# nordmtr/quantpy

Hardware: AMD Instinct MI355X
Metric: state reconstructions/sec (3-qubit MLE) (higher is better)
Workload: dtype f64

## Files before the change

quantpy_amd/csrc/qt_linesearch.h:

```cpp
#pragma once
#include <math.h>

#if defined(__HIPCC__)
#include <hip/hip_runtime.h>
#define QT_HD __host__ __device__ __forceinline__
#else
#define QT_HD inline
#endif

namespace qt {

enum LsResult : int { LS_EVAL = 0, LS_ACCEPT = 1, LS_FAIL = 2 };

struct LineSearch {
  double phi0, old_phi0, derphi0;
  int mode;
  int brackt, stage, evals;
  double gtest, width, width1, stx, fx, gx, sty, fy, gy, stmin, stmax;
  double alpha0, alpha1, phi_a0, phi_a1, derphi_a0;
  int it;
  double a_lo, a_hi, phi_lo, phi_hi, derphi_lo, phi_rec, a_rec;
  int zi;

  static constexpr double C1 = 1e-4, C2 = 0.9, AMAX = 1e100, AMIN = 1e-100, XTOL = 1e-14;
// ... 183 lines not shown
    }
    if (brackt) {
      if (fabs(sty - stx) >= 0.66 * width1) stp = stx + 0.5 * (sty - stx);
      width1 = width;
      width = fabs(sty - stx);
      stmin = dmin(stx, sty);
      stmax = dmax(stx, sty);
    } else {
      stmin = stp + 1.1 * (stp - stx);
      stmax = stp + 4.0 * (stp - stx);
    }
    stp = dmin(dmax(stp, AMIN), AMAX);
    if ((brackt && (stp <= stmin || stp >= stmax)) || (brackt && stmax - stmin <= XTOL * stmax)) stp = stx;
    if (!isfinite(stp)) return LS_FAIL;
    if (evals >= 99) return LS_FAIL;
    *next = stp;
    return LS_EVAL;
  }

  QT_HD static double cubicmin(double a, double fa, double fpa, double b, double fb, double c, double fc) {
    const double C = fpa, db = b - a, dc = c - a;
    const double denom = (db * dc) * (db * dc) * (db - dc);
    if (denom == 0.0) return NAN;
    const double t0 = fb - fa - C * db, t1 = fc - fa - C * dc;
    double A = dc * dc * t0 - db * db * t1;
    double B = -(dc * dc * dc) * t0 + db * db * db * t1;
    A /= denom;
    B /= denom;
    const double radical = B * B - 3.0 * A * C;
    if (!(radical >= 0.0) || A == 0.0) return NAN;
    const double x = a + (-B + sqrt(radical)) / (3.0 * A);
    return isfinite(x) ? x : NAN;
  }

  QT_HD static double quadmin(double a, double fa, double fpa, double b, double fb) {
    const double db = b - a;
    if (db == 0.0) return NAN;
    const double B = (fb - fa - fpa * db) / (db * db);
    if (B == 0.0) return NAN;
    const double x = a - fpa / (2.0 * B);
    return isfinite(x) ? x : NAN;
  }

  QT_HD int zoom_begin(double alo, double ahi, double plo, double phi_h, double dlo, double* next) {
    mode = 2;
    a_lo = alo; a_hi = ahi; phi_lo = plo; phi_hi = phi_h; derphi_lo = dlo;
    phi_rec = phi0;
    a_rec = 0.0;
    zi = 0;
    return zoom_propose(next);
  }

  QT_HD int zoom_propose(double* next) {
    const double dalpha = a_hi - a_lo;
    double a = a_lo, b = a_hi;
    if (dalpha < 0.0) { a = a_hi; b = a_lo; }
    double aj = NAN;
    bool need_quad = true;
    if (zi > 0) {
      const double cchk = 0.2 * dalpha;
      aj = cubicmin(a_lo, phi_lo, derphi_lo, a_hi, phi_hi, a_rec, phi_rec);
      need_quad = isnan(aj) || aj > b - cchk || aj < a + cchk;
    }
    if (need_quad) {
      const double qchk = 0.1 * dalpha;
      aj = quadmin(a_lo, phi_lo, derphi_lo, a_hi, phi_hi);
      if (isnan(aj) || aj > b - qchk || aj < a + qchk) aj = a_lo + 0.5 * dalpha;
    }
    *next = aj;
    return LS_EVAL;
  }

  QT_HD int advance_fallback(double stp, double f, double g, double* next) {
    if (mode == 1) {
      phi_a1 = f;
      const double derphi_a1 = g;
      if (alpha1 == 0.0 || alpha0 > AMAX) return LS_FAIL;
      if (phi_a1 > phi0 + C1 * alpha1 * derphi0 || (phi_a1 >= phi_a0 && it > 0))
        return zoom_begin(alpha0, alpha1, phi_a0, phi_a1, derphi_a0, next);
      if (fabs(derphi_a1) <= -C2 * derphi0) return LS_ACCEPT;
      if (derphi_a1 >= 0.0) return zoom_begin(alpha1, alpha0, phi_a1, phi_a0, derphi_a1, next);
      const double alpha2 = dmin(2.0 * alpha1, AMAX);
      alpha0 = alpha1;
      alpha1 = alpha2;
      phi_a0 = phi_a1;
      derphi_a0 = derphi_a1;
      ++it;
      if (it >= 10) mode = 3;
      *next = alpha1;
      return LS_EVAL;
    }
    if (mode == 3) return LS_ACCEPT;
    const double a_j = stp, phi_aj = f, derphi_aj = g;
    if (phi_aj > phi0 + C1 * a_j * derphi0 || phi_aj >= phi_lo) {
      phi_rec = phi_hi; a_rec = a_hi;
      a_hi = a_j; phi_hi = phi_aj;
    } else {
      if (fabs(derphi_aj) <= -C2 * derphi0) return LS_ACCEPT;
      if (derphi_aj * (a_hi - a_lo) >= 0.0) {
        phi_rec = phi_hi; a_rec = a_hi;
        a_hi = a_lo; phi_hi = phi_lo;
      } else {
        phi_rec = phi_lo; a_rec = a_lo;
      }
      a_lo = a_j; phi_lo = phi_aj; derphi_lo = derphi_aj;
    }
    ++zi;
    if (zi > 10) return LS_FAIL;
    return zoom_propose(next);
  }
};


enum TrialStatus : int {
  TRIAL_OK = 0,
  TRIAL_NOT_PD = 1,
  TRIAL_LINESEARCH = 2,
  TRIAL_MAXITER = 3,
  TRIAL_NAN = 4,
  TRIAL_SHOTS = 5
};

QT_HD int bfgs_eval_cap(int max_iter) { return (max_iter + 2) * 130; }

QT_HD double bfgs_rho(double ys) { return ys == 0.0 ? 1000.0 : 1.0 / ys; }

QT_HD bool bfgs_step_exit(double gnorm, double gtol, double stp, double pnorm2, double fk, int kiter, int max_iter,
                          int* status) {
  if (gnorm <= gtol) return true;
  if (stp * sqrt(pnorm2) <= 0.0) return true;
  if (!isfinite(fk)) {
    *status = TRIAL_LINESEARCH;
    return true;
  }
  return !(gnorm > gtol && kiter < max_iter);
}

QT_HD int bfgs_final_status(int status, int kiter, int max_iter, double gn, double fk, double xn) {
  if (status != TRIAL_OK) return status;
  if (kiter >= max_iter) return TRIAL_MAXITER;
  if (gn != gn || fk != fk || xn != xn) return TRIAL_NAN;
  return TRIAL_OK;
}

QT_HD int mle_start_status(bool shots_ok, bool ok, bool iterate, int max_iter, double gnorm, double fk, bool xnan) {
  if (!shots_ok) return TRIAL_SHOTS;
  if (!ok) return TRIAL_NOT_PD;
  if (iterate) return TRIAL_OK;
  if (0 >= max_iter) return TRIAL_MAXITER;
  if (gnorm != gnorm || fk != fk || xnan) return TRIAL_NAN;
  return TRIAL_OK;
}

}
```

quantpy_amd/csrc/qt_mle_small.h:

```cpp
#pragma once
#include <hip/hip_runtime.h>
#include <stdint.h>

#include <type_traits>

#include "qt_linesearch.h"
#include "qt_small.h"

namespace qt {

template <int NQ, bool GENERIC>
constexpr bool kStartBallots = NQ == 3 && !GENERIC && kLaneLeftovers;
template <int G>
__device__ __forceinline__ double start_norm_ballots(double gk, double gtol, bool& above) {
  const bool nan = group_any<G>(gk != gk);
  above = !nan && group_any<G>(fabs(gk) > gtol);
  return nan ? __builtin_nan("") : 0.0;
}

template <int NQ, bool GENERIC>
__global__ void __launch_bounds__(256) __attribute__((amdgpu_waves_per_eu(4))) k_mle_start(const int64_t* __restrict__ counts, const void* image, const double* Ns, int B, int M, int extra,
                                                   int max_iter, double gtol, typename MleArgs<GENERIC>::type pv0, int init, EstOut rho,
                                                   int32_t* __restrict__ nit_out, int32_t* __restrict__ nfev_out,
                                                   double* __restrict__ fun_out, int32_t* __restrict__ status_out,
// ... 235 lines not shown
    return -q;
  }
};

template <int NQ, class C>
__device__ __forceinline__ void bfgs_iterate(const C& c, bool mine, double xk, double gk,
                                             double fk, int b, int max_iter, double gtol, EstOut rho,
                                             int32_t* __restrict__ nit_out, int32_t* __restrict__ nfev_out,
                                             double* __restrict__ fun_out, int32_t* __restrict__ status_out) {
  DenseH<NQ> dir(c);
  LineSearch ls;
  bfgs_loop<NQ>(c, dir, ls, mine, xk, gk, fk, b, max_iter, gtol, rho, nit_out, nfev_out, fun_out, status_out);
}

template <int NQ, int LP = 0, class C>
__device__ __forceinline__ void bfgs_iterate_2l(const C& c, bool mine, double xk, double gk,
                                                double fk, int b, int max_iter, double gtol, EstOut rho,
                                                int32_t* __restrict__ nit_out, int32_t* __restrict__ nfev_out,
                                                double* __restrict__ fun_out, int32_t* __restrict__ status_out,
                                                double* __restrict__ pairs) {
  TwoLoop<NQ, LP> dir(c, pairs, b, max_iter);
  static_assert(sizeof(LineSearch) <= LineSearch::SLOTS * sizeof(double), "LDS slot of the line-search state");
  LineSearch& ls = *reinterpret_cast<LineSearch*>(c.extra());
  bfgs_loop<NQ>(c, dir, ls, mine, xk, gk, fk, b, max_iter, gtol, rho, nit_out, nfev_out, fun_out, status_out);
}

#ifndef QT_BFGS_WAVES
#define QT_BFGS_WAVES 2
#endif
template <int NQ, bool GENERIC>
__global__ void __launch_bounds__(256) __attribute__((amdgpu_waves_per_eu(QT_BFGS_WAVES))) k_mle_bfgs(const int64_t* __restrict__ counts, const void* image, const double* Ns, int B, int M, int extra, int max_iter,
                                                  double gtol, typename MleArgs<GENERIC>::type pv0, EstOut rho, int32_t* __restrict__ nit_out,
                                                  int32_t* __restrict__ nfev_out, double* __restrict__ fun_out,
                                                  int32_t* __restrict__ status_out, const double* __restrict__ ws_x,
                                                  const double* __restrict__ ws_g, const double* __restrict__ ws_f,
                                                  const int32_t* __restrict__ ws_active, double* __restrict__ pairs) {
  using S = Small<NQ>;
  constexpr int D = S::D;
  bool live;
  const int b = S::trial_index(B, &live);
  const bool mine = live && ws_active[b] != 0;
  if (!__syncthreads_or(mine)) return;
  extern __shared__ __attribute__((aligned(16))) double smem[];
  std::conditional_t<GENERIC, typename S::Ctx, typename S::template CtxSV<0>> c;
  const int bb = live ? b : B - 1;
  const auto pv = mle_front(pv0, image, Ns, M, extra);
  if constexpr (GENERIC) {
    S::make_ctx(c, smem, pv);
    S::load_freq(c, counts + (size_t)bb * pv.M);
  } else {
    typename S::Prefetch pf;
    S::prefetch_counts(pf, counts + (size_t)bb * pv.M, pv);
    S::take_coefs(c, pv);
    S::make_ctx(c, smem, pv, pf);
    S::load_freq(c, pf);
  }
  const double xk = mine ? ws_x[(size_t)b * D + c.l] : (c.l < S::d ? 1.0 : 0.0);
  const double gk = mine ? ws_g[(size_t)b * D + c.l] : 0.0;
  const double fk = mine ? ws_f[b] : 0.0;
  if constexpr (NQ == 3)
    bfgs_iterate_2l<NQ>(c, mine, xk, gk, fk, b, max_iter, gtol, rho, nit_out, nfev_out, fun_out, status_out, pairs);
  else
    bfgs_iterate<NQ>(c, mine, xk, gk, fk, b, max_iter, gtol, rho, nit_out, nfev_out, fun_out, status_out);
}

constexpr int kFusedLdsPairs = 24;
constexpr int kFusedHwLdsPairs = 16;

template <int NQ, bool GENERIC, bool HW = false>
__device__ __forceinline__ void mle_fused_body(const typename MleArgs<GENERIC>::type& pv, const int64_t* __restrict__ counts, int B, int init,
                                               int max_iter, double gtol, EstOut rho,
                                               int32_t* __restrict__ nit_out, int32_t* __restrict__ nfev_out,
                                               double* __restrict__ fun_out, int32_t* __restrict__ status_out,
                                               double* __restrict__ pairs) {
  using S = Small<NQ>;
  constexpr int D = S::D, G = S::G, d = S::d;
  extern __shared__ __attribute__((aligned(16))) double smem[];
  using Ctx = std::conditional_t<GENERIC, typename S::Ctx, typename S::template CtxSV<2>>;
  std::conditional_t<HW, typename S::template WithHelper<Ctx>, Ctx> c;
  [[maybe_unused]] typename S::HelperLink link;
  [[maybe_unused]] typename S::LateX late{false, 0.0, 0};
  [[maybe_unused]] int twin = 0;
  [[maybe_unused]] double* trial_sm = nullptr;
  bool live;
  const int b = S::trial_index(B, &live);
  const int bb = live ? b : B - 1;
  typename S::Prefetch pf;
  S::prefetch_counts(pf, counts + (size_t)bb * pv.M, pv);
  if constexpr (!GENERIC) S::take_coefs(c, pv);
  if constexpr (HW) {
    static_assert(NQ == 3, "one trial per wavefront");
    static_assert(S::HelperLink::doubles() <= kFusedHwLdsPairs * 2 * D, "the hand-off lives in the LDS pair store");
    int r1 = 6;
    if constexpr (GENERIC) r1 = pv.pr.R1;
    const int per_trial = S::trial_doubles(pv.M, r1);
    trial_sm = smem + S::table_doubles(pv.M, r1) + (threadIdx.x >> 6) * (per_trial + pv.extra);
    link.base = trial_sm + per_trial + LineSearch::SLOTS + 2 * max_iter;
    twin = __builtin_amdgcn_readfirstlane((int)threadIdx.y);
    link.pending = 0;
    if (!twin) link.reset();
    if (twin) __builtin_amdgcn_s_setprio(1);
    c.link = &link;
    c.xtra = trial_sm + per_trial;
    c.late = &late;
  }
  bool shots_ok;
  if constexpr (GENERIC) {
    S::template make_ctx<HW>(c, smem, pv, twin);
    QT_STAMP(0);
    shots_ok = S::load_freq(c, counts + (size_t)bb * pv.M, &pf);
  } else {
    S::template make_ctx<true, HW>(c, smem, pv, pf, twin);
    QT_STAMP(0);
    shots_ok = S::load_freq(c, pf);
  }
  QT_STAMP(1);
  int ok;
  double xk;
  typename S::StartPoint sp;
  [[maybe_unused]] cd lin;
  if (init == 0) {
    double bl;
    lin = S::lin_invert(c, bl);
    QT_STAMP(2);
    bool feasible = false;
    if constexpr (HW) {
      if (twin) {
        if (!S::twin_lift(c, link, lin, sp.rho)) {
          S::HelperLink::publish(link.gone(), 1);
          return;
        }
        sp.lscale = 1.0;
        link.pending = 1;
        feasible = true;
      }
    }
    if (!feasible) sp.rho = S::template make_feasible<!HW>(c, lin, &xk, &ok, &sp.lscale);
    if constexpr (HW) {
      if (!twin && __builtin_amdgcn_readfirstlane(link.pending)) {
        int r1 = 6;
        if constexpr (GENERIC) r1 = pv.pr.R1;
        double* twin_sm = smem + S::twin_offset(pv.M, r1, pv.extra) + (threadIdx.x >> 6) * S::trial_doubles(pv.M, r1);
        S::sweep_for(c, link, sp.rho, reinterpret_cast<cd*>(twin_sm + S::oB));
        S::HelperLink::publish(link.gone(), 1);
        return;
      }
    }
  } else {
    sp.rho = cd{c.i == c.j ? 1.0 / d : 0.0, 0.0};
    sp.lscale = 1.0;
    xk = S::cholesky_param(c, sp.rho, ok);
  }
  QT_STAMP(8);
  double fk, gk;
  cd rho_l;
  [[maybe_unused]] typename S::DeferredValue dv;
  bool evaluate = true;
  if constexpr (HW) {
    if (__builtin_amdgcn_readfirstlane(link.pending)) {
      if constexpr (GENERIC) S::template nll_grad<false, decltype(c), true>(c, 0.0, fk, gk, &rho_l, true, &sp);
      else S::template nll_grad<true, decltype(c), true>(c, 0.0, fk, gk, &rho_l, true, &sp, &dv);
      xk = late.x;
      ok = late.ok;
      const bool got = __builtin_amdgcn_readfirstlane((int)late.got) != 0;
      if (!got) xk = S::cholesky_param(c, sp.rho, ok);
      ok = __builtin_amdgcn_readfirstlane(ok);
      evaluate = !got || !ok;
      if (!ok) {
        sp.rho = S::psd_project(c, lin, 1e-15);
        xk = S::cholesky_param(c, sp.rho, ok);
      }
    }
  }
  if (evaluate) {
    if constexpr (GENERIC) S::nll_grad(c, xk, fk, gk, &rho_l, true, &sp);
    else S::template nll_grad<true>(c, xk, fk, gk, &rho_l, true, &sp, &dv);
  }
  double gnorm;
  bool iterate;
  if constexpr (kStartBallots<NQ, GENERIC>) {
    bool above;
    gnorm = start_norm_ballots<G>(gk, gtol, above);
    QT_STAMP(9);
    iterate = live && shots_ok && ok && above && (0 < max_iter);
  } else {
    gnorm = gmax<G>(fabs(gk));
    QT_STAMP(9);
    iterate = live && shots_ok && ok && (gnorm > gtol) && (0 < max_iter);
  }
  if constexpr (!GENERIC) fk = S::value_if_needed(c, dv, iterate || fun_out != nullptr);
  S::emit(c, rho, b, live && !iterate, rho_l);
  const int status = mle_start_status(shots_ok, ok, iterate, max_iter, gnorm, fk, group_any<G>(xk != xk));
  if (live && !iterate && c.l == 0) store_trial(b, 0, ok ? 1 : 0, fk, status, nit_out, nfev_out, fun_out, status_out);
  QT_STAMP(10);
  if (!__any(iterate)) return;
  if (!iterate) {
    xk = (c.l < d) ? 1.0 : 0.0;
    gk = 0.0;
    fk = 0.0;
  }
  if constexpr (HW) link.await_gone();
  if constexpr (NQ == 3)
    bfgs_iterate_2l<NQ, HW ? kFusedHwLdsPairs : kFusedLdsPairs>(c, iterate, xk, gk, fk, b, max_iter, gtol, rho, nit_out, nfev_out, fun_out,
                                              status_out, pairs);
  else
    bfgs_iterate<NQ>(c, iterate, xk, gk, fk, b, max_iter, gtol, rho, nit_out, nfev_out, fun_out, status_out);
}

template <int NQ, bool GENERIC>
__global__ void __launch_bounds__(256) k_mle_fused(const int64_t* __restrict__ counts, const void* image, const double* Ns, int B, int M, int extra, int max_iter,
                                                   double gtol, typename MleArgs<GENERIC>::type pv, EstOut rho, int32_t* __restrict__ nit_out,
                                                   int32_t* __restrict__ nfev_out, double* __restrict__ fun_out,
                                                   int32_t* __restrict__ status_out, double* __restrict__ pairs) {
  mle_fused_body<NQ, GENERIC>(mle_front(pv, image, Ns, M, extra), counts, B, 0, max_iter, gtol, rho, nit_out, nfev_out, fun_out, status_out, pairs);
}
template <int NQ, bool GENERIC>
__global__ void __launch_bounds__(256) k_mle_fused_mixed(const int64_t* __restrict__ counts, const void* image, const double* Ns, int B, int M, int extra,
                                                         int max_iter, double gtol, typename MleArgs<GENERIC>::type pv, EstOut rho,
                                                         int32_t* __restrict__ nit_out, int32_t* __restrict__ nfev_out,
                                                         double* __restrict__ fun_out, int32_t* __restrict__ status_out,
                                                         double* __restrict__ pairs) {
  mle_fused_body<NQ, GENERIC>(mle_front(pv, image, Ns, M, extra), counts, B, 1, max_iter, gtol, rho, nit_out, nfev_out, fun_out, status_out, pairs);
}

template <int NQ, bool GENERIC>
__global__ void __launch_bounds__(512) k_mle_fused_hw(const int64_t* __restrict__ counts, const void* image, const double* Ns, int B, int M, int extra, int max_iter,
                                                      double gtol, typename MleArgs<GENERIC>::type pv, EstOut rho, int32_t* __restrict__ nit_out,
                                                      int32_t* __restrict__ nfev_out, double* __restrict__ fun_out,
                                                      int32_t* __restrict__ status_out, double* __restrict__ pairs) {
  mle_fused_body<NQ, GENERIC, true>(mle_front(pv, image, Ns, M, extra), counts, B, 0, max_iter, gtol, rho, nit_out, nfev_out, fun_out, status_out, pairs);
}

}
```

quantpy_amd/csrc/qt_small.h:

```cpp
#pragma once
#include <hip/hip_runtime.h>
#include <stdint.h>

#include "qt_args.h"
#include "qt_wave.h"

namespace qt {

constexpr bool kLiftSingleNegative = true;

#ifndef QT_LANE_INT_FRONT
#define QT_LANE_INT_FRONT 1
#endif
#ifndef QT_LANE_LEFTOVERS
#define QT_LANE_LEFTOVERS 1
#endif
constexpr bool kLaneLeftovers = QT_LANE_LEFTOVERS != 0;

template <int NQ>
struct Small {
  static constexpr int d = 1 << NQ;
  static constexpr int D = d * d;
  static constexpr int G = D;
  static constexpr int TPW = 64 / G;
  static constexpr int WPB = 4;
  static constexpr int NT = 64 * WPB;
  static constexpr int TPB = TPW * WPB;
  static constexpr int T = d * (d - 1) / 2;
  static constexpr int LD = d == 8 ? 9 : d;
  static constexpr int MAT = 2 * LD * d;
  static constexpr int oA = 0;
  static constexpr int oB = oA + MAT;
  static constexpr int oVec = oB + MAT;
  static constexpr int oLam = oVec + D + 2;
  static constexpr int oM = oLam + 2 * ((d + 1) / 2);
  __host__ __device__ static bool v_on_rbuf(int M) { return ((M + 1) & ~1) >= MAT; }
  __host__ __device__ static int v_offset(int M, int R1) {
    const int Mp = (M + 1) & ~1;
    return v_on_rbuf(M) ? oM : oM + (R1 > 0 ? 3 : 2) * Mp;
  }
  __host__ __device__ static int trial_doubles(int M, int R1 = 0) {
    const int Mp = (M + 1) & ~1;
    return oM + (R1 > 0 ? 3 : 2) * Mp + (v_on_rbuf(M) ? 0 : MAT);
  }
  __host__ __device__ static int ipow_h(int b, int e) {
    int r = 1;
    for (int t = 0; t < e; ++t) r *= b;
    return r;
  }
  __host__ __device__ static int fwd_ints(int R1) {
    int t = 0;
    for (int q = 1; q <= NQ; ++q) t += ipow_h(R1, q) << (2 * (NQ - q));
    return t;
  }
  __host__ __device__ static int bwd_ints(int R1) {
    int t = 0;
    for (int q = 1; q <= NQ; ++q) t += ipow_h(R1, q - 1) << (2 * (NQ - q + 1));
    return t;
  }
  __host__ __device__ static int table_ints(int M, int R1) { return (fwd_ints(R1) + bwd_ints(R1) + M + 1) & ~1; }
  __host__ __device__ static int table_doubles(int M, int R1) {
    return R1 > 0 ? (table_ints(M, R1) / 2 + ((M + 1) & ~1) + 8 * R1) : 0;
  }
  __host__ __device__ static size_t lds_bytes(int M, int R1 = 0, int extra = 0) {
    return ((size_t)table_doubles(M, R1) + (size_t)TPB * (trial_doubles(M, R1) + extra)) * sizeof(double);
  }
  __host__ __device__ static int twin_offset(int M, int R1, int extra) {
    return table_doubles(M, R1) + TPB * (trial_doubles(M, R1) + extra);
  }
  __host__ __device__ static size_t lds_bytes_twin(int M, int R1, int extra) {
    return lds_bytes(M, R1, extra) + (size_t)TPB * trial_doubles(M, R1) * sizeof(double);
  }

  struct Ctx {
    int l, i, j, e;
    double* sm;
    const int *tfwd, *tbwd, *trmap;
    const double* twrow;
    const double *ttab, *ptab;
    int M, Mp;
    PovmView pv;
    int xm, zm, ny;
    int pi, pj, pkind;
    int src_re, src_im;
    __device__ __forceinline__ cd* A() const { return reinterpret_cast<cd*>(sm + oA); }
    __device__ __forceinline__ cd* Bm() const { return reinterpret_cast<cd*>(sm + oB); }
    __device__ __forceinline__ cd* V() const { return reinterpret_cast<cd*>(sm + v_offset(M, pv.pr.enabled ? pv.pr.R1 : 0)); }
    __device__ __forceinline__ double* vec() const { return sm + oVec; }
    __device__ __forceinline__ double* lam() const { return sm + oLam; }
    __device__ __forceinline__ double* rbuf() const { return sm + oM; }
    __device__ __forceinline__ double* freq() const { return sm + oM + Mp; }
    __device__ __forceinline__ double* bufB() const { return sm + oM + 2 * Mp; }
    __device__ __forceinline__ const double* tabT() const { return ttab; }
    __device__ __forceinline__ const double* tabP() const { return ptab; }
    __device__ __forceinline__ bool prod() const { return pv.pr.enabled != 0; }
    __device__ __forceinline__ double* extra() const { return sm + trial_doubles(M, pv.pr.enabled ? pv.pr.R1 : 0); }
    static constexpr bool kGeneric = true;
    static constexpr int kLaneTables = 0;
    static constexpr bool kHelper = false;
    __device__ __forceinline__ static constexpr int verdict_load() { return 0; }
    __device__ __forceinline__ static constexpr bool abandoned(int) { return false; }
    __device__ __forceinline__ int R1() const { return pv.pr.R1; }
    __device__ __forceinline__ bool uniform() const { return pv.pr.uniform != 0; }
    __device__ __forceinline__ bool pairedT() const { return pv.pr.pairedT != 0; }
    __device__ __forceinline__ bool pairedP() const { return pv.pr.pairedP != 0; }
    __device__ __forceinline__ double wuni() const { return pv.pr.wuni; }
    __device__ __forceinline__ double jtol2() const { return pv.jtol2; }
    __device__ __forceinline__ double cT(int k) const { return pv.pr.cT[k]; }
    __device__ __forceinline__ double cP(int k) const { return pv.pr.cP[k]; }
  };
  template <int LT>
  struct CtxSV {
    static constexpr bool VC = LT == 2;
    int l, i, j, e;
    double* sm;
    const int* tfwd;
    const double *ttab, *ptab;
    int M, Mp;
    SpecArgs a;
    int xm, zm, ny;
    int pi, pj, pkind;
    int src_re, src_im;
    int bslot;
    double kT[12], kP[12];
    uint32_t mpack[2];
    const double* mterm[VC ? d : 1];
    uint32_t msign[VC ? d : 1];
    uint32_t bflip[VC ? 4 : 1];
    static constexpr int kLaneTables = LT;
    __device__ __forceinline__ cd* A() const { return reinterpret_cast<cd*>(sm + oA); }
    __device__ __forceinline__ cd* Bm() const { return reinterpret_cast<cd*>(sm + oB); }
    __device__ __forceinline__ cd* V() const { return reinterpret_cast<cd*>(sm + v_offset(M, 6)); }
    __device__ __forceinline__ double* vec() const { return sm + oVec; }
    __device__ __forceinline__ double* lam() const { return sm + oLam; }
    __device__ __forceinline__ double* rbuf() const { return sm + oM; }
    __device__ __forceinline__ double* freq() const { return sm + oM + Mp; }
    __device__ __forceinline__ double* bufB() const { return sm + oM + 2 * Mp; }
    __device__ __forceinline__ const double* tabT() const { return ttab; }
    __device__ __forceinline__ const double* tabP() const { return ptab; }
    __device__ __forceinline__ double* extra() const { return sm + trial_doubles(M, 6); }
    static constexpr bool kGeneric = false;
    static constexpr bool kHelper = false;
    __device__ __forceinline__ static constexpr int verdict_load() { return 0; }
    __device__ __forceinline__ static constexpr bool abandoned(int) { return false; }
    __device__ __forceinline__ static constexpr bool prod() { return true; }
    __device__ __forceinline__ static constexpr int R1() { return 6; }
    __device__ __forceinline__ static constexpr bool uniform() { return true; }
    __device__ __forceinline__ static constexpr bool pairedT() { return true; }
    __device__ __forceinline__ static constexpr bool pairedP() { return true; }
    __device__ __forceinline__ double wuni() const { return a.wuni; }
    __device__ __forceinline__ double jtol2() const { return a.jtol2; }
    __device__ __forceinline__ double cT(int k) const { return kT[k]; }
    __device__ __forceinline__ double cP(int k) const { return kP[k]; }
  };
  using CtxS = CtxSV<1>;
  __device__ __forceinline__ static double pin_vgpr(double x) {
    asm volatile("" : "+v"(x));
    return x;
  }
  template <bool GENERIC, class = void>
  struct CtxOf {
    using type = Ctx;
  };
  template <class X>
  struct CtxOf<false, X> {
    using type = CtxSV<1>;
  };
  __host__ __device__ static int image_last_ints(int M) { return (M + 3) & ~3; }
  __host__ __device__ static int image_chunks(int M) { return image_last_ints(M) / 4 + 2 * 24 / 2; }

// ... 1077 lines not shown
    const int* verdict;
    __device__ __forceinline__ cd* A() const { return image; }
    __device__ __forceinline__ cd* Bm() const { return factor; }
    __device__ __forceinline__ cd* V() const { return second; }
    __device__ __forceinline__ int verdict_load() const {
      return __hip_atomic_load(verdict, __ATOMIC_RELAXED, __HIP_MEMORY_SCOPE_WORKGROUP);
    }
    __device__ __forceinline__ static bool abandoned(int v) {
      v = __builtin_amdgcn_readfirstlane(v);
      return v != HelperLink::kPending && v != HelperLink::kGo;
    }
  };
  struct LateX {
    bool got;
    double x;
    int ok;
  };
  template <class Base>
  struct WithHelper : Base {
    HelperLink* link;
    LateX* late;
    double* xtra;
    __device__ __forceinline__ double* extra() const { return xtra; }
    static constexpr bool kHelper = true;
  };
  __device__ __forceinline__ static void param_owner(int l, int& pi, int& pj, int& pkind) {
    const bool diag = l < d, imag = l >= d + T;
    const int t = l - d - (imag ? T : 0);
    int ii = 1;
#pragma unroll
    for (int k = 2; k < d; ++k) ii += t >= (k * (k - 1)) / 2;
    pkind = diag ? 0 : imag ? 2 : 1;
    pi = diag ? l : ii;
    pj = diag ? l : t - (ii * (ii - 1)) / 2;
  }
  template <class C>
  __device__ static bool twin_lift(const C& t, const HelperLink& k, cd lin, cd& proj) {
    static_assert(G == 64, "one trial per wavefront");
    CtxH c = side_ctx(t, k, t.Bm());
    proj = cd{0.0, 0.0};
    const bool lifted = __builtin_amdgcn_readfirstlane((int)lift_single_negative<true>(c, lin, d - 1, 1e-15, proj, nullptr)) != 0;
    QT_STAMP(6);
    if (HelperLink::template poll<1>(k.verdict(), HelperLink::kPending, HelperLink::kHelperPolls) != HelperLink::kGo) return false;
    QT_STAMP(7);
    if (!HelperLink::claim(k.verdict(), HelperLink::kGo, HelperLink::kClaimed)) return false;
    if (!lifted) {
      HelperLink::publish(k.lifted(), HelperLink::kRefused);
      return false;
    }
    k.result()[c.e] = proj;
    HelperLink::publish(k.lifted(), HelperLink::kLifted);
    return true;
  }
  template <class C>
  __device__ static void sweep_for(const C& t, const HelperLink& k, cd proj, cd* L) {
    CtxH c = side_ctx(t, k, L);
    int ok2;
    const double x2 = cholesky_param(c, proj, ok2);
    k.x()[c.l] = x2;
    if (c.l == 0) *k.ok() = ok2;
    HelperLink::publish(k.done(), 1);
    QT_STAMP(7);
  }
  template <class C>
  __device__ __forceinline__ static CtxH side_ctx(const C& t, const HelperLink& k, cd* L) {
    CtxH c;
    c.l = t.l;
    c.i = t.i;
    c.j = t.j;
    c.e = t.e;
    c.pi = t.pi;
    c.pj = t.pj;
    c.pkind = t.pkind;
    c.image = t.A();
    c.second = t.V();
    c.factor = L;
    c.verdict = k.verdict();
    return c;
  }

  template <bool NATURAL = false, class C>
  __device__ static bool lift_single_negative(const C& c, cd r, int kneg, double eps, cd& out,
                                              const cd* inverse = nullptr) {
    static_assert(G == 64, "one trial per wavefront: the flags below are wave-uniform");
    cd* Ai = c.A();
    cd* Vi = c.V();
    const int i = c.i, j = c.j;
    if (i == j) r.im = 0.0;
    cd b = r;
    if (inverse) b = *inverse;
    auto eliminate = [&](int p) {
      Ai[c.e] = b;
      const double piv = readlane_f64(b.re, p * d + p);
      wave_sync();
      const cd bip = Ai[i * LD + p], bpj = Ai[p * LD + j];
      wave_sync();
      double inv = __builtin_amdgcn_rcp(piv);
      inv = fma(inv, fma(-piv, inv, 1.0), inv);
      inv = fma(inv, fma(-piv, inv, 1.0), inv);
      const cd t{bpj.re * inv, bpj.im * inv};
      const cd e = cmul(bip, t);
      cd nb{b.re - e.re, b.im - e.im};
      if (j == p) nb = cd{-bip.re * inv, -bip.im * inv};
      if (i == p) nb = (j == p) ? cd{inv, 0.0} : t;
      b = nb;
    };
    if constexpr (NATURAL) {
      if (!inverse) {
#pragma unroll
        for (int p = 0; p < d; ++p) eliminate(p);
      }
    } else {
#pragma unroll 1
      for (int s = inverse ? d : 0; s < d; ++s) eliminate(s < kneg ? s : (s < d - 1 ? s + 1 : kneg));
    }
    QT_STAMP(4);
    b = cscale(b, fast_rsqrt(gsum<G>(b.re * b.re + b.im * b.im)));
    bool certified = false, called_off = false;
#pragma unroll 1
    for (int k = 1;; ++k) {
      Ai[c.e] = b;
      wave_sync();
      [[maybe_unused]] const int verdict = c.verdict_load();
      cd n{0.0, 0.0}, n2{0.0, 0.0};
#pragma unroll
      for (int q = 0; q < d; q += 2) {
        const cd u = Ai[i * LD + q], v = Ai[j * LD + q];
        n.re = fma(u.re, v.re, fma(u.im, v.im, n.re));
        n.im = fma(u.im, v.re, fma(-u.re, v.im, n.im));
        if (q + 1 < d) {
          const cd u2 = Ai[i * LD + q + 1], v2 = Ai[j * LD + q + 1];
          n2.re = fma(u2.re, v2.re, fma(u2.im, v2.im, n2.re));
          n2.im = fma(u2.im, v2.re, fma(-u2.re, v2.im, n2.im));
        }
      }
      n = cadd(n, n2);
      wave_sync();
      called_off = c.abandoned(verdict);
      const double pur = gsum<G>(n.re * n.re + n.im * n.im);
      b = cscale(n, fast_rsqrt(pur));
      const double defect = 1.0 - pur;
      QT_STAMP_VAL(20, k);
#ifdef QT_PHASE_TIMING
      if (k <= 5) QT_STAMP(25 + k);
#endif
      if (called_off | certified | (k == 7) | ((k == 3) & !(defect < 0.05))) break;
      certified = defect < 1e-7;
    }
    QT_STAMP(5);
    if (called_off || !certified) return false;
    if (i == j) b.im = 0.0;
    b = cscale(b, 1.0 / gtrace<G>(i == j, b.re));
    const double lam = gsum<G>(r.re * b.re + r.im * b.im);
    if (!(lam < eps)) return false;
    Ai[c.e] = r;
    Vi[c.e] = b;
    wave_sync();
    cd q{-lam * b.re, -lam * b.im};
#pragma unroll
    for (int k = 0; k < d; ++k) {
      const cd u = Ai[i * LD + k], v = Vi[j * LD + k];
      q.re = fma(u.re, v.re, fma(u.im, v.im, q.re));
      q.im = fma(u.im, v.re, fma(-u.re, v.im, q.im));
    }
    wave_sync();
    const double res2 = gsum<G>(q.re * q.re + q.im * q.im);
    const double nrm2 = gsum<G>(r.re * r.re + r.im * r.im);
    if (!(res2 <= 1e-26 * nrm2)) return false;
    const double w = eps - lam;
    cd o{fma(w, b.re, r.re), fma(w, b.im, r.im)};
    const double tr = gtrace<G>(i == j, o.re);
    out = cd{o.re / tr, o.im / tr};
    return true;
  }

  template <bool SPEC = false, class C>
  __device__ static cd make_feasible(const C& c, cd r, double* xl, int* ok_out, double* lscale_out = nullptr) {
    int ok, neg, kneg;
    cd spec_inv{0.0, 0.0};
    double x = cholesky_param<SPEC && G == 64>(c, r, ok, &neg, &kneg, &spec_inv);
    QT_STAMP(3);
    cd out{0.0, 0.0};
    double lscale = 1.0;
    auto pd_epilogue = [&]() {
      const double tr = gtrace<G>(c.i == c.j, r.re);
      out = cd{r.re / tr, r.im / tr};
      const double rst = tr > 0.0 ? fast_rsqrt(tr) : 1.0 / sqrt(tr);
      x = x * rst;
      lscale = rst;
    };
    const bool all_pd = __all(ok);
    [[maybe_unused]] bool go = false;
    if constexpr (C::kHelper) {
      go = kLiftSingleNegative && !all_pd && __builtin_amdgcn_readfirstlane(neg) == 1 &&
           __builtin_amdgcn_readfirstlane(kneg) == d - 1;
      c.link->decide(go);
    }
    if (G < 64 || all_pd || (!xl && lscale_out)) pd_epilogue();
    if (!all_pd) {
      cd proj;
      bool lifted = false;
      [[maybe_unused]] bool refused = false;
      if constexpr (C::kHelper) {
        if (go) {
          const int came = c.link->await_lift(c.e, proj);
          QT_STAMP(31);
          if (came == HelperLink::kLifted) {
            QT_STAMP(6);
            if (lscale_out) *lscale_out = 1.0;
            return proj;
          }
          refused = came == HelperLink::kRefused;
        }
      }
      if constexpr (G == 64) {
        if (kLiftSingleNegative && !refused && __builtin_amdgcn_readfirstlane(neg) == 1) {
          const int kn = __builtin_amdgcn_readfirstlane(kneg);
          lifted = __builtin_amdgcn_readfirstlane(
                       (int)lift_single_negative(c, r, kn, 1e-15, proj, SPEC && kn == d - 1 ? &spec_inv : nullptr)) != 0;
        }
      }
      if (!lifted) proj = psd_project(c, r, 1e-15);
      QT_STAMP(6);
      int ok2 = 1;
      double x2 = xl ? cholesky_param(c, proj, ok2) : 0.0;
      if (lifted && xl && !__all(ok2 || ok)) {
        proj = psd_project(c, r, 1e-15);
        x2 = cholesky_param(c, proj, ok2);
      }
      QT_STAMP(7);
      if (xl) lscale = 1.0;
      if (!ok) {
        out = proj;
        x = x2;
        ok = ok2;
      }
    }
    if (xl) *xl = x;
    if (ok_out) *ok_out = ok;
    if (lscale_out) *lscale_out = lscale;
    return out;
  }

  template <class C>
  __device__ static cd build_llh(const C& c, double xl, double& tr) {
    double* vx = c.vec();
    cd* L = c.Bm();
    vx[c.l] = xl;
    tr = gsum<G>(xl * xl);
    wave_sync();
    const int i = c.i, j = c.j;
    L[c.e] = cd{vx[c.src_re], vx[c.src_im]};
    wave_sync();
    cd m{0.0, 0.0};
#pragma unroll
    for (int k = 0; k < d; ++k) {
      const cd u = L[i * LD + k], v = L[j * LD + k];
      m.re = fma(u.re, v.re, fma(u.im, v.im, m.re));
      m.im = fma(u.im, v.re, fma(-u.re, v.im, m.im));
    }
    return m;
  }

  struct StartPoint {
    cd rho;
    double lscale;
  };
  template <bool DEFER = false, class C, bool LATE = false>
  __device__ static void nll_grad(const C& c, double xl, double& f, double& gl, cd* rho_l = nullptr,
                                  bool want_grad = true, const StartPoint* start = nullptr, DeferredValue* dv = nullptr) {
    static_assert(!DEFER || !C::kGeneric, "the deferred value needs the compile-time row count of the specialised shape");
    double tr;
    QT_STAMP(11);
    cd m;
    if constexpr (LATE) {
      m = start->rho;
    } else if (start) {
      tr = gsum<G>(xl * xl);
      m = cd{start->rho.re * tr, start->rho.im * tr};
    } else {
      m = build_llh(c, xl, tr);
    }
    QT_STAMP(12);
    cd* A = c.A();
    const cd rho_e = start ? start->rho : cd{m.re / tr, m.im / tr};
    if (rho_l) *rho_l = rho_e;
    A[c.e] = rho_e;
    wave_sync();
    const double bl = bloch_of(c, A);
    QT_STAMP(13);
    double* vec = c.vec();
    if constexpr (!(NQ == 3 && C::kLaneTables != 0 && kLaneLeftovers)) {
      vec[c.l] = bl;
      wave_sync();
    }
    double fpart = 0.0;
    const double* fr = c.freq();
    double* rb = c.rbuf();
    double wl;
    if (c.prod()) {
      const int R1 = c.R1();
      const bool paired = c.pairedT() != 0;
      const int* tab = c.tfwd;
      const double* in = vec;
#pragma unroll
      for (int q = 1; q < NQ; ++q) {
        const int stride = 1 << (2 * (NQ - q));
        const int n_out = ipow(R1, q) * stride;
        double* out = ((NQ - 1 - q) & 1) ? rb : c.bufB();
        if (paired) {
          paired_forward(c, q, in, out);
        } else if constexpr (C::kGeneric) {
          stage<true>(c, c.tabT(), tab, n_out, stride, in, out);
          tab += n_out;
        }
        in = out;
      }
      QT_STAMP(14);
      if constexpr (DEFER) {
        stage_n_log<true, true, true>(c, tab, in, fr, rb, dv);
      } else if constexpr (!C::kGeneric) {
        fpart = stage_n_log<true, true>(c, tab, in, fr, rb);
      } else {
        if (!paired) fpart = stage_n_log<false, false>(c, tab, in, fr, rb);
        else if (c.uniform()) fpart = stage_n_log<true, true>(c, tab, in, fr, rb);
        else fpart = stage_n_log<true, false>(c, tab, in, fr, rb);
      }
      if constexpr (!DEFER) f = -gsum<G>(fpart);
      wave_sync();
      QT_STAMP(15);
      if (!want_grad) return;
      wl = prod_backward<false>(c, rb);
      QT_STAMP(16);
    } else if constexpr (C::kGeneric) {
      for (int m0 = 0; m0 < c.M; m0 += G) {
        const int mm = m0 + c.l;
        if (mm < c.M) {
          const double pe = row_dot(c, c.pv.AwT, mm, vec) * d + 1e-10;
          fpart += fr[mm] * fast_log(pe);
          rb[mm] = fr[mm] * recip_nr(pe);
        }
      }
      f = -gsum<G>(fpart);
      wave_sync();
      if (!want_grad) return;
      wl = col_dot(c, c.pv.Aw, rb);
    }
    const double tr_g_rho = -(double)d * gsum<G>(wl * bl);
    vec[c.l] = wl;
    wave_sync();
    cd g = matrix_of(c, vec);
    QT_STAMP(17);
    if constexpr (LATE) {
      LateX& lx = *c.late;
      lx.x = 1.0;
      lx.ok = 0;
      lx.got = c.link->collect(c.l, lx.x, lx.ok);
      xl = lx.x;
      tr = gsum<G>(xl * xl);
      QT_STAMP(25);
    }
    g.re = -g.re;
    g.im = -g.im;
    if (c.i == c.j) g.re -= tr_g_rho;
    g.re /= tr;
    g.im /= tr;
    A[c.e] = g;
    wave_sync();
    const cd* L = c.Bm();
    cd q{0.0, 0.0};
#pragma unroll
    for (int k = 0; k < d; ++k) {
      const cd u = A[c.pi * LD + k], v = L[k * LD + c.pj];
      q.re = fma(u.re, v.re, fma(-u.im, v.im, q.re));
      q.im = fma(u.re, v.im, fma(u.im, v.re, q.im));
    }
    gl = 2.0 * (c.pkind == 2 ? q.im : q.re);
    if (start) gl *= start->lscale;
    wave_sync();
    QT_STAMP(18);
  }

  template <class C>
  __device__ __forceinline__ static double hs_to_centre(const C& c, cd r, const double* __restrict__ centre) {
    const double2 cc = *reinterpret_cast<const double2*>(centre + 2 * c.l);
    const cd dl{r.re - cc.x, r.im - cc.y};
    const int src = (int)(threadIdx.x & 63) - c.l + c.j * d + c.i;
    const cd dt{__shfl(dl.re, src, 64), __shfl(dl.im, src, 64)};
    const cd t = hs_term(dl, dt);
    const double sr = gsum<G>(t.re);
    const double si = gsum<G>(t.im);
    const double v = sqrt(hypot(sr, si)) / sqrt(2.0);
    return v < 1e-15 ? 0.0 : v;
  }
  template <class C>
  __device__ __forceinline__ static void emit(const C& c, const EstOut& o, int b, bool store, cd r) {
    if (o.dist) {
      const double v = hs_to_centre(c, r, o.centre_of(b, 2 * D));
      if (store && c.l == 0) o.dist[b] = v;
    }
    if (store && o.rho) {
      double* out = o.rho + ((size_t)b * D + c.l) * 2;
      out[0] = r.re;
      out[1] = r.im;
    }
  }
};


template <int NQ>
__global__ void __launch_bounds__(256) k_lin_batch(PovmView pv, const int64_t* __restrict__ counts, int B, int physical,
                                                   EstOut rho, double* __restrict__ bloch_out,
                                                   int32_t* __restrict__ status) {
  using S = Small<NQ>;
  extern __shared__ __attribute__((aligned(16))) double smem[];
  typename S::Ctx c;
  bool live;
  const int b = S::trial_index(B, &live);
  const int bb = live ? b : B - 1;
  typename S::Prefetch pf;
  S::prefetch_counts(pf, counts + (size_t)bb * pv.M, pv);
  S::make_ctx(c, smem, pv);
  QT_STAMP(0);
  const bool shots_ok = S::load_freq(c, counts + (size_t)bb * pv.M, &pf);
  QT_STAMP(1);
  double bl;
  cd r = S::lin_invert(c, bl);
  QT_STAMP(2);
  if (physical) r = S::make_feasible(c, r, nullptr, nullptr);
  QT_STAMP(9);
  S::emit(c, rho, b, live, r);
  if (live) {
    if (bloch_out) bloch_out[(size_t)b * S::D + c.l] = bl;
    if (status && c.l == 0) status[b] = !shots_ok ? 5 : (r.re == r.re) ? 0 : 4;
  }
}

template <int NQ>
__global__ void __launch_bounds__(256) k_chol_param(PovmView pv, const double* __restrict__ rho, int B,
                                                    double* __restrict__ x, int32_t* __restrict__ status) {
  using S = Small<NQ>;
  extern __shared__ __attribute__((aligned(16))) double smem[];
  typename S::Ctx c;
  S::make_ctx(c, smem, pv);
  bool live;
  const int b = S::trial_index(B, &live);
  const int bb = live ? b : B - 1;
  const double* in = rho + ((size_t)bb * S::D + c.l) * 2;
  int ok;
  const double xl = S::cholesky_param(c, cd{in[0], in[1]}, ok);
  if (live) {
    x[(size_t)b * S::D + c.l] = xl;
    if (status && c.l == 0) status[b] = ok ? 0 : 1;
  }
}

template <int NQ>
__global__ void __launch_bounds__(256) k_chol_unparam(PovmView pv, const double* __restrict__ x, int B,
                                                      double* __restrict__ llh) {
  using S = Small<NQ>;
  extern __shared__ __attribute__((aligned(16))) double smem[];
  typename S::Ctx c;
  S::make_ctx(c, smem, pv);
  bool live;
  const int b = S::trial_index(B, &live);
  const int bb = live ? b : B - 1;
  double tr;
  const cd m = S::build_llh(c, x[(size_t)bb * S::D + c.l], tr);
  if (live) {
    double* out = llh + ((size_t)b * S::D + c.l) * 2;
    out[0] = m.re;
    out[1] = m.im;
  }
}

enum Metric { kMetricTrace = 0, kMetricInfidelity = 1 };

template <int NQ>
__global__ void __launch_bounds__(256) k_psd_sqrt(const double* __restrict__ centres, int G, double jtol2,
                                                  double* __restrict__ roots) {
  using S = Small<NQ>;
  __shared__ __attribute__((aligned(16))) double smem[S::TPB * S::kMetricDoubles];
  typename S::CtxM c;
  S::make_ctx_metric(c, smem, jtol2);
  bool live;
  const int g = S::trial_index(G, &live);
  const int gg = live ? g : G - 1;
  const double* in = centres + ((size_t)gg * S::D + c.l) * 2;
  const cd s = S::psd_sqrt(c, cd{in[0], in[1]});
  if (live) {
    double* out = roots + ((size_t)g * S::D + c.l) * 2;
    out[0] = s.re;
    out[1] = s.im;
  }
}

template <int NQ, int METRIC>
__global__ void __launch_bounds__(256) k_metric_dist(const double* __restrict__ rho, int B,
                                                     const double* __restrict__ centres, int G, int g0, double jtol2,
                                                     double* __restrict__ dist) {
  using S = Small<NQ>;
  __shared__ __attribute__((aligned(16))) double smem[S::TPB * S::kMetricDoubles];
  typename S::CtxM c;
  S::make_ctx_metric(c, smem, jtol2);
  bool live;
  const int b = S::trial_index(B, &live);
  const int bb = live ? b : B - 1;
  const double* in = rho + ((size_t)bb * S::D + c.l) * 2;
  const double* cen = centre_of(centres, G, g0, bb, 2 * S::D) + 2 * c.l;
  const cd r{in[0], in[1]}, q{cen[0], cen[1]};
  const double v = METRIC == kMetricTrace ? S::trace_dist(c, r, q) : S::infidelity(c, r, q);
  if (live && c.l == 0) dist[b] = v;
}

template <int NQ>
__global__ void __launch_bounds__(256) k_nll_batch(PovmView pv, const double* __restrict__ x,
                                                   const int64_t* __restrict__ counts, int B, double* __restrict__ f,
                                                   double* __restrict__ grad) {
  using S = Small<NQ>;
  extern __shared__ __attribute__((aligned(16))) double smem[];
  typename S::Ctx c;
  S::make_ctx(c, smem, pv);
  bool live;
  const int b = S::trial_index(B, &live);
  const int bb = live ? b : B - 1;
  S::load_freq(c, counts + (size_t)bb * pv.M);
  double fv, gl;
  S::nll_grad(c, x[(size_t)bb * S::D + c.l], fv, gl);
  if (live) {
    if (c.l == 0) f[b] = fv;
    if (grad) grad[(size_t)b * S::D + c.l] = gl;
  }
}

}
```

Before: 116.7 million.

## Emit start outputs early and merge single-negative lift exit checks

The MLE start kernel now writes rho and the default trial scalars right after the feasible starting point is built, before the gradient evaluation. The final stores are skipped when the early values already match the final status. This is meant to overlap global stores with compute and shorten the tail. The single-negative lift routine also computes its output and residual check unconditionally, combining two exit branches into one. That removes divergent early returns at the cost of some extra work, and it adds redundant speculative stores that are overwritten whenever a trial iterates.

Measured after the change: 119.1 million (median of 6 runs). 1.02x the previous value.

```diff
diff --git a/quantpy_amd/csrc/qt_linesearch.h b/quantpy_amd/csrc/qt_linesearch.h
--- a/quantpy_amd/csrc/qt_linesearch.h
+++ b/quantpy_amd/csrc/qt_linesearch.h
@@ -359,4 +359,10 @@
   return TRIAL_OK;
 }
 
-}
+QT_HD bool mle_early_scalars_final(bool shots_ok, bool ok, bool iterate, int max_iter, double gnorm, double fk,
+                                   bool xnan, bool fun_wanted) {
+  if (fun_wanted) return false;
+  return ok && mle_start_status(shots_ok, ok, iterate, max_iter, gnorm, fk, xnan) == TRIAL_OK;
+}
+
+}
diff --git a/quantpy_amd/csrc/qt_mle_small.h b/quantpy_amd/csrc/qt_mle_small.h
--- a/quantpy_amd/csrc/qt_mle_small.h
+++ b/quantpy_amd/csrc/qt_mle_small.h
@@ -411,6 +411,13 @@
     xk = S::cholesky_param(c, sp.rho, ok);
   }
   QT_STAMP(8);
+  [[maybe_unused]] bool early_rho = false, early_scalars = false;
+  if constexpr (kEarlyOutputs) {
+    S::emit_rho(c, rho, b, live, sp.rho);
+    early_rho = true;
+    early_scalars = fun_out == nullptr;
+    if (early_scalars && live && c.l == 0) store_trial(b, 0, 1, 0.0, TRIAL_OK, nit_out, nfev_out, nullptr, status_out);
+  }
   double fk, gk;
   cd rho_l;
   [[maybe_unused]] typename S::DeferredValue dv;
@@ -428,6 +435,7 @@
       if (!ok) {
         sp.rho = S::psd_project(c, lin, 1e-15);
         xk = S::cholesky_param(c, sp.rho, ok);
+        early_rho = false;
       }
     }
   }
@@ -448,9 +456,16 @@
     iterate = live && shots_ok && ok && (gnorm > gtol) && (0 < max_iter);
   }
   if constexpr (!GENERIC) fk = S::value_if_needed(c, dv, iterate || fun_out != nullptr);
-  S::emit(c, rho, b, live && !iterate, rho_l);
-  const int status = mle_start_status(shots_ok, ok, iterate, max_iter, gnorm, fk, group_any<G>(xk != xk));
-  if (live && !iterate && c.l == 0) store_trial(b, 0, ok ? 1 : 0, fk, status, nit_out, nfev_out, fun_out, status_out);
+  if constexpr (kEarlyOutputs) {
+    S::emit_dist(c, rho, b, live && !iterate, rho_l);
+    if (!early_rho) S::emit_rho(c, rho, b, live && !iterate, rho_l);
+  } else {
+    S::emit(c, rho, b, live && !iterate, rho_l);
+  }
+  const bool xnan = group_any<G>(xk != xk);
+  const int status = mle_start_status(shots_ok, ok, iterate, max_iter, gnorm, fk, xnan);
+  const bool stored = early_scalars && mle_early_scalars_final(shots_ok, ok, iterate, max_iter, gnorm, fk, xnan, fun_out != nullptr);
+  if (live && !iterate && c.l == 0 && !stored) store_trial(b, 0, ok ? 1 : 0, fk, status, nit_out, nfev_out, fun_out, status_out);
   QT_STAMP(10);
   if (!__any(iterate)) return;
   if (!iterate) {
diff --git a/quantpy_amd/csrc/qt_small.h b/quantpy_amd/csrc/qt_small.h
--- a/quantpy_amd/csrc/qt_small.h
+++ b/quantpy_amd/csrc/qt_small.h
@@ -16,6 +16,14 @@
 #define QT_LANE_LEFTOVERS 1
 #endif
 constexpr bool kLaneLeftovers = QT_LANE_LEFTOVERS != 0;
+#ifndef QT_LIFT_ONE_EXIT
+#define QT_LIFT_ONE_EXIT 1
+#endif
+#ifndef QT_EARLY_OUTPUTS
+#define QT_EARLY_OUTPUTS 1
+#endif
+constexpr bool kLiftOneExit = QT_LIFT_ONE_EXIT != 0;
+constexpr bool kEarlyOutputs = QT_EARLY_OUTPUTS != 0;
 
 template <int NQ>
 struct Small {
@@ -1399,6 +1407,26 @@
     if (i == j) b.im = 0.0;
     b = cscale(b, 1.0 / gtrace<G>(i == j, b.re));
     const double lam = gsum<G>(r.re * b.re + r.im * b.im);
+    if constexpr (kLiftOneExit) {
+      Ai[c.e] = r;
+      Vi[c.e] = b;
+      const double w = eps - lam;
+      const cd o{fma(w, b.re, r.re), fma(w, b.im, r.im)};
+      const double tr = gtrace<G>(i == j, o.re);
+      out = cd{o.re / tr, o.im / tr};
+      wave_sync();
+      cd q{-lam * b.re, -lam * b.im};
+#pragma unroll
+      for (int k = 0; k < d; ++k) {
+        const cd u = Ai[i * LD + k], v = Vi[j * LD + k];
+        q.re = fma(u.re, v.re, fma(u.im, v.im, q.re));
+        q.im = fma(u.im, v.re, fma(-u.re, v.im, q.im));
+      }
+      wave_sync();
+      const double res2 = gsum<G>(q.re * q.re + q.im * q.im);
+      const double nrm2 = gsum<G>(r.re * r.re + r.im * r.im);
+      return (lam < eps) & (res2 <= 1e-26 * nrm2);
+    }
     if (!(lam < eps)) return false;
     Ai[c.e] = r;
     Vi[c.e] = b;
@@ -1646,6 +1674,21 @@
       const double v = hs_to_centre(c, r, o.centre_of(b, 2 * D));
       if (store && c.l == 0) o.dist[b] = v;
     }
+    if (store && o.rho) {
+      double* out = o.rho + ((size_t)b * D + c.l) * 2;
+      out[0] = r.re;
+      out[1] = r.im;
+    }
+  }
+  template <class C>
+  __device__ __forceinline__ static void emit_dist(const C& c, const EstOut& o, int b, bool store, cd r) {
+    if (o.dist) {
+      const double v = hs_to_centre(c, r, o.centre_of(b, 2 * D));
+      if (store && c.l == 0) o.dist[b] = v;
+    }
+  }
+  template <class C>
+  __device__ __forceinline__ static void emit_rho(const C& c, const EstOut& o, int b, bool store, cd r) {
     if (store && o.rho) {
       double* out = o.rho + ((size_t)b * D + c.l) * 2;
       out[0] = r.re;
```
